# juanmc2005/diart

Measured on AMD Instinct MI355X. Metric: real-time-factor xRT streams/GPU @500ms step, higher is better.
Workload: dtype f16x3

## Files before the change

### diart_amd/_lib.py

```python
from __future__ import annotations

import ctypes as C
import os
from pathlib import Path
from typing import Optional

EXPERIMENTS = os.environ.get("DZ_EXPERIMENTS", "0") not in ("", "0")
_LIB_PATH = Path(__file__).resolve().parent / ("libdiart_amd_exp.so" if EXPERIMENTS else "libdiart_amd.so")
_lib: Optional[C.CDLL] = None

c_float_p = C.POINTER(C.c_float)
c_double_p = C.POINTER(C.c_double)
c_int_p = C.POINTER(C.c_int)
vp = C.c_void_p


class SincNetWeights(C.Structure):
    _fields_ = [("wav_gamma", C.c_float), ("wav_beta", C.c_float)] + [
        (n, vp) for n in ("filt", "in0_g", "in0_b", "w1", "b1", "in1_g", "in1_b",
                          "w2", "b2", "in2_g", "in2_b", "w1_split", "w2_split", "filt_split")]


class SegWeights(C.Structure):
    _fields_ = [("sinc", SincNetWeights), ("wih", vp * 4), ("bih", vp * 4), ("whh", vp * 4),
# ... 155 lines not shown
    "dz_tail_step": (C.c_int, [vp, vp, C.c_double, C.c_double, vp, vp, vp, vp, vp, C.c_int, vp]),
    "dz_tail_step_batch": (C.c_int, [C.POINTER(vp), C.c_int, vp, vp, vp, vp, vp, vp, vp, vp,
                                     C.c_int, vp, C.c_int]),
    "dz_file_step_batch": (C.c_int, [C.POINTER(vp), C.POINTER(vp), C.c_int, vp, vp, vp, C.c_int, C.c_int, vp, C.c_int,
                                     C.c_int, vp, C.c_double, vp, C.c_int, vp, vp, C.c_int]),
    "dz_rows_repeat": (C.c_int, [vp, vp, C.c_longlong, C.c_int, C.c_int, vp, c_int_p]),
    "dz_k_convgemm": (C.c_int, [vp, vp, vp]),
    "dz_k_gemm_f32": (C.c_int, [vp, vp, vp]),
    "dz_k_gemm_split": (C.c_int, [vp, vp, vp]),
    "dz_k_gemm_pre": (C.c_int, [vp, vp, vp]),
    "dz_k_mlp_head": (C.c_int, [vp, vp, C.c_longlong, vp, vp, vp, vp, vp, vp, C.c_int, C.c_int, C.c_int, C.c_int,
                                C.c_int, C.c_float, C.c_float, vp, vp, vp]),
    "dz_k_seg_head": (C.c_int, [vp, vp, vp, vp, C.c_int, C.c_int, C.c_int, C.c_int, C.c_int, vp, C.c_float,
                                C.c_float, C.c_int, vp, vp]),
    "dz_k_conv_pool": (C.c_int, [vp, vp, vp]),
    "dz_k_convgemm_ntile": (C.c_int, [C.c_int]),
    "dz_k_wave_stats": (C.c_int, [vp, vp, C.c_longlong, C.c_int, C.c_int, vp, vp]),
    "dz_k_sinc_conv0": (C.c_int, [vp, vp, C.c_longlong, C.c_int, C.c_int, vp, C.c_float,
                                  C.c_float, vp, vp, vp, vp]),
    "dz_k_sinc_conv0_split": (C.c_int, [vp, vp, C.c_longlong, C.c_int, C.c_int, vp, C.c_float,
                                        C.c_float, vp, vp, vp, vp]),
    "dz_k_conv0_split_ntile": (C.c_int, [C.c_int]),
    "dz_k_finalize_norm": (C.c_int, [vp, vp, C.c_int, C.c_int, C.c_int, C.c_int, vp, vp, vp, vp, vp]),
    "dz_k_lstm": (C.c_int, [vp, vp, vp, vp, C.c_int, C.c_int, vp]),
    "dz_k_lstm_mfma": (C.c_int, [vp, vp, vp, vp, C.c_int, C.c_int, C.c_int, C.c_int, vp]),
    "dz_k_lstm_planes": (C.c_int, [vp, vp, vp, vp, C.c_int, vp, C.c_longlong, C.c_int, C.c_int, vp]),
    "dz_k_stats_pool": (C.c_int, [vp, vp, C.c_int, C.c_int, C.c_int, vp, C.c_int, C.c_int,
                                  C.c_int, vp, C.c_int, vp]),
    "dz_k_powerset": (C.c_int, [vp, vp, C.c_int, C.c_int, C.c_int, vp, vp]),
    "dz_k_conv2d": (C.c_int, [vp, vp, vp, vp, vp, vp, vp, C.c_int, C.c_int, C.c_int, C.c_int, C.c_int, C.c_int,
                              C.c_int, C.c_int, vp]),
    "dz_k_ttn_depthwise": (C.c_int, [vp, vp, C.c_int, vp, C.c_int, vp, C.c_int, C.c_int, C.c_int, C.c_int, vp, vp, vp]),
}


EXPERIMENT_SIGNATURES = {
    "dz_k_gemm_g2": (C.c_int, [vp, vp, C.c_int, vp]),
    "dz_k_gemm_g3": (C.c_int, [vp, vp, C.c_int, vp]),
    "dz_k_conv_pool_debug": (C.c_int, [vp]),
    "dz_sinc_conv0_pair": (C.c_int, [vp, vp, vp, C.c_longlong, C.c_int, vp, vp, vp, vp]),
    "dz_k_sinc_conv0_pair": (C.c_int, [vp, vp, C.c_longlong, C.c_int, C.c_int, vp, vp, vp, C.c_float, C.c_float, vp, vp,
                                       vp, vp, vp]),
}


class ConvGemmDesc(C.Structure):
    _fields_ = [(n, vp) for n in ("X", "W", "bias", "e0", "e1", "nscale", "nshift", "Y", "partials")] + [
        (n, C.c_int) for n in ("B", "Tin", "Tout", "Cin", "taps", "dil", "K", "Kpad", "Npad",
                               "Nstore", "ldx", "ldy", "nld", "Tstore")] + [
        ("xbs", C.c_longlong), ("ybs", C.c_longlong), ("norm_on_load", C.c_int), ("epi", C.c_int),
        ("ksplit", C.c_int), ("ysplit", C.c_longlong), ("agroup", C.c_int), ("pad", C.c_int),
        ("X2", vp), ("rowbias", vp), ("Wsplit", vp), ("Xsplit", vp), ("xplane", C.c_longlong),
        ("Ysplit", vp), ("yplane", C.c_longlong), ("npart", vp), ("ngamma", vp), ("nbeta", vp),
        ("npart_tiles", C.c_int), ("npart_T", C.c_int), ("oflag", vp), ("Tdev", vp)]


(EPI_BIAS, EPI_BIAS_LEAKY, EPI_BIAS_SIGMOID, EPI_TDNN, EPI_POOL3, EPI_BIAS_RELU, EPI_RELU_BN,
 EPI_RELU_BN_TANH) = range(8)


class DiartAmdError(RuntimeError):
    pass


def lib_path() -> Path:
    return _LIB_PATH


def load() -> C.CDLL:
    global _lib
    if _lib is None:
        if not _LIB_PATH.exists():
            raise DiartAmdError(
                f"{_LIB_PATH} not found: build it with `python -m diart_amd.build` "
                "(hipcc, gfx950).  diart_amd has no CPU fallback.")
        lib = C.CDLL(str(_LIB_PATH))
        for name, (res, args) in SIGNATURES.items():
            fn = getattr(lib, name)
            fn.restype = res
            fn.argtypes = args
        if lib.dz_has_experiments():
            for name, (res, args) in EXPERIMENT_SIGNATURES.items():
                fn = getattr(lib, name)
                fn.restype = res
                fn.argtypes = args
        elif EXPERIMENTS:
            raise DiartAmdError(f"DZ_EXPERIMENTS=1 but {_LIB_PATH} is not an experiments build")
        sizes = (C.c_int * 5)()
        lib.dz_abi_struct_sizes(C.byref(sizes))
        mine = [C.sizeof(t) for t in (SincNetWeights, SegWeights, EmbWeights, EcapaWeights, ConvGemmDesc)]
        if list(sizes) != mine:
            raise DiartAmdError(f"{_LIB_PATH} was built from a different include/diart_amd.h: struct sizes "
                                f"{list(sizes)} (library) vs {mine} (this binding); rebuild it")
        for name, struct in (("dz_wsp", WspWeights), ("dz_sbx", SbxWeights), ("dz_ttn", TtnWeights)):
            size = getattr(lib, f"{name}_abi_size")()
            if size != C.sizeof(struct):
                raise DiartAmdError(f"{_LIB_PATH} was built from a different include/diart_amd.h: sizeof({name}_weights) "
                                    f"{size} (library) vs {C.sizeof(struct)} (this binding); rebuild it")
        _lib = lib
    return _lib


def experiments() -> bool:
    return bool(load().dz_has_experiments())


def exp_env(name: str, default: str) -> str:
# ... 47 lines not shown
```

### diart_amd/csrc/dz_embed.h

```cpp
#pragma once
#include "dz_common.h"

#include <string.h>
#include <new>

inline bool dz_conv_pool_enabled() {
    const char* v = dz_exp_env("DZ_CONV_POOL");
    return !(v && v[0] == '0');
}

struct DzGemm {
    DzConvGemm p;
    const void *wsplit, *wfrag;
    int tag, units;

    static DzGemm dense(const dz_layer& L, const float* X, int ldx, long long rows, int Cin, float* Y, int ldy,
                        int Nstore, int epi) {
        return conv1d(L, X, ldx, 1, (int)rows, Cin, Y, ldy, Nstore, epi).xstride(0, 0);
    }
    static DzGemm conv1d(const dz_layer& L, const float* X, int ldx, int B, int T, int Cin, float* Y, int ldy,
                         int Nstore, int epi) {
        DzGemm g;
        memset(&g, 0, sizeof(g));
        g.wsplit = L.wsplit;
        g.tag = -1;
        DzConvGemm& p = g.p;
        p.X = X; p.W = L.w; p.bias = L.b; p.e0 = L.s; p.e1 = L.h; p.Y = Y;
        p.B = B; p.Tin = p.Tout = p.Tstore = T; p.Cin = Cin; p.taps = 1; p.dil = 1; p.K = p.Kpad = Cin;
        p.Npad = p.Nstore = Nstore; p.ldx = ldx; p.ldy = ldy; p.epi = epi;
        return g.xstride((long long)T * ldx, (long long)T * ldy);
    }
    DzGemm& xstride(long long xbs, long long ybs) { p.xbs = xbs; p.ybs = ybs; return *this; }
    DzGemm& taps(int n, int dil, int pad) {
        p.taps = n; p.dil = dil; p.pad = pad; p.K = n * p.Cin;
        p.Tout = p.Tstore = pad ? p.Tin : p.Tin - (n - 1) * dil;
        return *this;
    }
    DzGemm& padded(int Kpad, int Npad) { p.Kpad = Kpad; p.Npad = Npad; return *this; }
    DzGemm& x2(const float* X2) { p.X2 = X2; return *this; }
    DzGemm& rowbias(const float* rb) { p.rowbias = rb; return *this; }
    DzGemm& splitk(int n, long long ysplit) { p.ksplit = n; p.ysplit = ysplit; return *this; }
    DzGemm& xplanes(const void* Xs, long long xplane) { p.Xsplit = Xs; p.xplane = Xs ? xplane : 0; return *this; }
    DzGemm& planes_out(void* Ys, long long yplane) { p.Ysplit = Ys; p.yplane = Ys ? yplane : 0; return *this; }
    DzGemm& norm_partials(const float* part, int tiles, int T, const float* gamma, const float* beta, int nld) {
        p.npart = part; p.npart_tiles = tiles; p.npart_T = T; p.ngamma = gamma; p.nbeta = beta;
        p.nld = nld; p.norm_on_load = 1;
        return *this;
    }
    DzGemm& norm_scaled(const float* nscale, const float* nshift, int nld) {
        p.nscale = nscale; p.nshift = nshift; p.nld = nld; p.norm_on_load = 1;
        return *this;
    }
    DzGemm& pool3(float* partials) {
        p.partials = partials; p.Tstore = p.Tout / 3; p.ybs = (long long)p.Tstore * p.ldy;
        return *this;
    }
    DzGemm& frag(const void* f) { wfrag = f; return *this; }
    DzGemm& tdev(const int* T) { p.Tdev = T; return *this; }
    DzGemm& prof(int t, int u) { tag = t; units = u; return *this; }

    int run(hipStream_t st) {
        DzProfScope ps(tag, units);
        if (p.Xsplit) {
            p.X = p.W = nullptr;
            p.Wsplit = wsplit;
            return dz_launch_gemm_pre(p, st);
        }
        if (wsplit && p.ksplit <= 1) {
            p.Wsplit = wsplit;
            if (p.epi == DZ_EPI_POOL3)
                return dz_conv_pool_enabled() ? dz_launch_conv_pool(p, st, wfrag) : dz_launch_gemm_split(p, st);
            p.Npad = (p.Npad + 127) / 128 * 128;
            return dz_launch_gemm_split(p, st);
        }
        DZ_REQUIRE(p.Ysplit == nullptr, "DzGemm: plane output asked of a layer that is not on the split-f16 path");
        return dz_launch_convgemm(p, st);
    }
    int run_pooled(const DzPoolFuse& q, hipStream_t st) {
        DzProfScope ps(tag, units);
        p.X = p.W = nullptr;
        p.Wsplit = wsplit;
        return dz_launch_gemm_pre_pool(p, q, st);
    }
};

constexpr int DZ_TAG_OF_GEMM = -2;
inline int dz_splitk_linear(const dz_layer& L, const float* X, int rows, int Cin, int Kpad, int N, int nsplit,
                            float* parts, int finish, float* out, hipStream_t st, int tag = -1,
// ... 90 lines not shown
```

### diart_amd/csrc/k_gemm_pre.hip

```cpp
#include "dz_common.h"
#include <stdlib.h>
#include <type_traits>

namespace {

typedef _Float16 f16x8 __attribute__((ext_vector_type(8)));
typedef _Float16 f16x2 __attribute__((ext_vector_type(2)));
typedef float f32x16 __attribute__((ext_vector_type(16)));

constexpr int BM = 128, BN = 128, KT = 32;
constexpr int PLANE_B = 128 * 64;
constexpr int plane_a(int MW) { return 64 * MW * 64; }
constexpr int stage_bytes(int MW) { return 2 * plane_a(MW) + 2 * PLANE_B; }
constexpr size_t lds_bytes(int MW) { return 2 * (size_t)stage_bytes(MW) + 3 * BN * sizeof(float); }
constexpr int MW_BIG = 6;
constexpr float LO_UNSCALE = 1.f / 2048.f;

__device__ __forceinline__ float leaky(float v) { return fmaxf(v, v * DZ_LEAKY_SLOPE); }

constexpr int YT_PITCH = 132;
constexpr int POOL_PAR = BM * YT_PITCH * 4;
constexpr int POOL_WT = POOL_PAR + 3 * BN * 4;
constexpr int POOL_RED = POOL_WT + 4 * BM * 4;
constexpr int POOL_S0 = POOL_RED + 2 * 2 * 4 * BN * 4;
constexpr size_t POOL_LDS = POOL_S0 + 8 * 8 * 2 * 4 + 8 * 2 * 4;

template <int EPI, int MW, int MT, int NT, bool ILV = false, bool POOL = false>
__device__ __forceinline__ void gemm_pre_tile(const DzConvGemm& p, const int t0, const int n0, char* smem,
                                              const int flags = 0, const DzPoolFuse* q = nullptr) {
    constexpr int PLANE_A = plane_a(MW), STAGE = stage_bytes(MW), PAR_OFF = POOL ? POOL_PAR : 2 * STAGE;
    static_assert(!POOL || (MW == 2 && MT == 2 && NT == 2), "pooled epilogue: 128 x 128 tiles only");
    const int tid = threadIdx.x;
    const int w = __builtin_amdgcn_readfirstlane(tid >> 6), l = tid & 63;

    constexpr int PA = 2 * MT * MW, PB = 4 * NT, NWAVE = 2 * MW;
    constexpr int NWA = (NWAVE * PA + (PA + PB) / 2) / (PA + PB);
    constexpr int JMAX_A = (2 * PA + NWA - 1) / NWA, JMAX_B = (2 * PB + (NWAVE - NWA) - 1) / (NWAVE - NWA);
    constexpr int JMAX = JMAX_A > JMAX_B ? JMAX_A : JMAX_B;
    const bool isB = w >= NWA;
    const int rank = isB ? w - NWA : w, group = isB ? NWAVE - NWA : NWA, npc = isB ? PB : PA;
    const unsigned short* src = isB ? reinterpret_cast<const unsigned short*>(p.Wsplit)
                                    : reinterpret_cast<const unsigned short*>(p.Xsplit);
    const int prows = isB ? p.Npad : (int)((unsigned)p.xplane / (unsigned)p.ldx);
    const long long plane_el = isB ? (long long)p.Npad * p.Kpad : p.xplane;
    const unsigned nbytes = (unsigned)((long long)prows * (isB ? p.Kpad : p.ldx) * 2);
    const __amdgpu_buffer_rsrc_t rs_hi = __builtin_amdgcn_make_buffer_rsrc((void*)src, 0, nbytes, 0x00020000);
    const __amdgpu_buffer_rsrc_t rs_lo = __builtin_amdgcn_make_buffer_rsrc((void*)(src + plane_el), 0, nbytes, 0x00020000);
    const int voff0 = ((isB ? n0 : t0) + (l >> 2)) * 64 + (((l & 3) ^ ((l >> 4) & 3)) << 4);
    constexpr int vstep = 16 * 64;
    const int kb_bytes = prows * 64;
    const int dst0 = isB ? 2 * PLANE_A : 0, dplane = isB ? PLANE_B : PLANE_A;
    auto issue = [&](int kt, int stage) {
        int cblk = kt, tap = 0;
        if (p.taps > 1) {
            cblk = kt / p.taps;
            tap = kt - cblk * p.taps;
        }
        const int soff = isB ? (tap * (p.Cin >> 5) + cblk) * kb_bytes : cblk * kb_bytes + tap * p.dil * 64;
        char* dst = smem + stage * STAGE + dst0;
#pragma unroll
        for (int j = 0; j < JMAX; ++j) {
            const int q = rank + j * group;
            if (q >= 2 * npc) break;
            const int lo = q >= npc, i = q - lo * npc;
            __builtin_amdgcn_raw_ptr_buffer_load_lds(lo ? rs_lo : rs_hi,
                (__attribute__((address_space(3))) void*)(dst + lo * dplane + i * 1024), 16,
                voff0 + i * vstep, soff, 0, 0);
        }
    };

    const int li = l & 31, g = l >> 5;
    const int wm = w >> 1, wn = w & 1;
    const int sw = (li >> 2) & 3;
    int foff[2];
#pragma unroll
    for (int ks = 0; ks < 2; ++ks) foff[ks] = li * 64 + (((2 * ks + g) ^ sw) << 4);
    f32x16 accm[MT][NT], accx[MT][NT];
#pragma unroll
    for (int mt = 0; mt < MT; ++mt)
#pragma unroll
        for (int nt = 0; nt < NT; ++nt)
#pragma unroll
            for (int r = 0; r < 16; ++r) accm[mt][nt][r] = accx[mt][nt][r] = 0.f;

    auto compute = [&](int stage) {
        const char* st = smem + stage * STAGE;
        const char* sa = st + (wm * 32 * MT) * 64;
        const char* sb = st + 2 * PLANE_A + (wn * 32 * NT) * 64;
#pragma unroll
        for (int ks = 0; ks < 2; ++ks) {
            f16x8 ah[MT], al[MT], bh[NT], bl[NT];
#pragma unroll
            for (int t = 0; t < MT; ++t) {
                ah[t] = *reinterpret_cast<const f16x8*>(sa + t * 2048 + foff[ks]);
                al[t] = *reinterpret_cast<const f16x8*>(sa + PLANE_A + t * 2048 + foff[ks]);
            }
#pragma unroll
            for (int t = 0; t < NT; ++t) {
                bh[t] = *reinterpret_cast<const f16x8*>(sb + t * 2048 + foff[ks]);
                bl[t] = *reinterpret_cast<const f16x8*>(sb + PLANE_B + t * 2048 + foff[ks]);
            }
#pragma unroll
            for (int mt = 0; mt < MT; ++mt)
#pragma unroll
                for (int nt = 0; nt < NT; ++nt) {
                    accx[mt][nt] = __builtin_amdgcn_mfma_f32_32x32x16_f16(bh[nt], al[mt], accx[mt][nt], 0, 0, 0);
                    accm[mt][nt] = __builtin_amdgcn_mfma_f32_32x32x16_f16(bh[nt], ah[mt], accm[mt][nt], 0, 0, 0);
                    accx[mt][nt] = __builtin_amdgcn_mfma_f32_32x32x16_f16(bl[nt], ah[mt], accx[mt][nt], 0, 0, 0);
                }
        }
    };

    const int nk = p.Kpad / KT;
    issue(0, 0);
    constexpr bool FULL = MW == 2 && MT == 2 && NT == 2;
    float* par = reinterpret_cast<float*>(smem + PAR_OFF);
    {
        constexpr bool AFF = EPI == DZ_EPI_TDNN || EPI == DZ_EPI_RELU_BN;
        const int which = tid >> 5, c4 = (tid & 31) * 4;
        if (which < (AFF ? 3 : 1)) {
            const float* src = which == 0 ? p.bias : which == 1 ? p.e0 : p.e1;
            f32x4 v = {0.f, 0.f, 0.f, 0.f};
            if (n0 + c4 + 3 < p.Npad) v = *reinterpret_cast<const f32x4*>(src + n0 + c4);
            *reinterpret_cast<f32x4*>(par + which * BN + c4) = v;
        }
    }
    if (FULL && ILV) {
        const int r2 = w & 1;
        char* const dbase = smem + dst0 + r2 * 1024;
        const int vofs = voff0 + r2 * vstep;
        int cblk = 0, tap = 0;
        const int tap_step = isB ? (p.Cin >> 5) * kb_bytes : p.dil * 64;
        auto advance = [&]() -> int {
            if (++tap == p.taps) { tap = 0; ++cblk; }
            return cblk * kb_bytes + tap * tap_step;
        };
        int soff_next = 0, stage_next = 0;
        const bool no_dma = flags & 2, no_rd = flags & 4;
        const bool skip_a = (flags & 32) && !isB;
        auto piece = [&](int j) {
            const int lo = j >= 4, i = r2 + 2 * (j & 3);
            (void)i;
            if (no_dma || (skip_a && tap != 0 && cblk > 0)) return;
            __builtin_amdgcn_raw_ptr_buffer_load_lds(lo ? rs_lo : rs_hi,
                (__attribute__((address_space(3))) void*)(dbase + stage_next * STAGE + lo * dplane + (j & 3) * 2048), 16,
                vofs + (j & 3) * 2 * vstep, soff_next, 0, 0);
        };
        const char* sa0 = smem + (wm * 64) * 64;
        const char* sb0 = smem + 2 * PLANE_A + (wn * 64) * 64;
#define DZ_RD(base, plane, t, ks) (*reinterpret_cast<const f16x8*>((no_rd ? smem : (base) + (plane) + (t) * 2048) + foff[ks]))
#define DZ_MM(mt, nt)                                                                                     \
    accx[mt][nt] = __builtin_amdgcn_mfma_f32_32x32x16_f16(bh[nt], al[mt], accx[mt][nt], 0, 0, 0);          \
    accm[mt][nt] = __builtin_amdgcn_mfma_f32_32x32x16_f16(bh[nt], ah[mt], accm[mt][nt], 0, 0, 0);          \
    accx[mt][nt] = __builtin_amdgcn_mfma_f32_32x32x16_f16(bl[nt], ah[mt], accx[mt][nt], 0, 0, 0)
#define DZ_PIN() __builtin_amdgcn_sched_barrier(0)
        auto body = [&](const int kt, auto more_c) {
            constexpr bool more = decltype(more_c)::value;
            asm volatile("s_waitcnt vmcnt(0) lgkmcnt(0)\n\ts_barrier" ::: "memory");
            soff_next = advance();
            stage_next = (kt + 1) & 1;
            const char* sa = sa0 + (kt & 1) * STAGE;
            const char* sb = sb0 + (kt & 1) * STAGE;
            f16x8 ah[2], al[2], bh[2], bl[2];
            bh[0] = DZ_RD(sb, 0, 0, 0); al[0] = DZ_RD(sa, PLANE_A, 0, 0); ah[0] = DZ_RD(sa, 0, 0, 0);
            bl[0] = DZ_RD(sb, PLANE_B, 0, 0);
            bh[1] = DZ_RD(sb, 0, 1, 0); bl[1] = DZ_RD(sb, PLANE_B, 1, 0);
            ah[1] = DZ_RD(sa, 0, 1, 0); al[1] = DZ_RD(sa, PLANE_A, 1, 0);
            DZ_PIN();
            accx[0][0] = __builtin_amdgcn_mfma_f32_32x32x16_f16(bh[0], al[0], accx[0][0], 0, 0, 0);
            accm[0][0] = __builtin_amdgcn_mfma_f32_32x32x16_f16(bh[0], ah[0], accm[0][0], 0, 0, 0);
            DZ_PIN();
            if (more) piece(0);
            DZ_PIN();
            accx[0][0] = __builtin_amdgcn_mfma_f32_32x32x16_f16(bl[0], ah[0], accx[0][0], 0, 0, 0);
            accx[0][1] = __builtin_amdgcn_mfma_f32_32x32x16_f16(bh[1], al[0], accx[0][1], 0, 0, 0);
            DZ_PIN();
            if (more) piece(1);
            DZ_PIN();
            accm[0][1] = __builtin_amdgcn_mfma_f32_32x32x16_f16(bh[1], ah[0], accm[0][1], 0, 0, 0);
            accx[0][1] = __builtin_amdgcn_mfma_f32_32x32x16_f16(bl[1], ah[0], accx[0][1], 0, 0, 0);
            DZ_PIN();
            if (more) piece(2);
            ah[0] = DZ_RD(sa, 0, 0, 1); al[0] = DZ_RD(sa, PLANE_A, 0, 1);
            DZ_PIN();
            accx[1][1] = __builtin_amdgcn_mfma_f32_32x32x16_f16(bh[1], al[1], accx[1][1], 0, 0, 0);
            accm[1][1] = __builtin_amdgcn_mfma_f32_32x32x16_f16(bh[1], ah[1], accm[1][1], 0, 0, 0);
            DZ_PIN();
            if (more) piece(3);
            DZ_PIN();
            accx[1][1] = __builtin_amdgcn_mfma_f32_32x32x16_f16(bl[1], ah[1], accx[1][1], 0, 0, 0);
            accx[1][0] = __builtin_amdgcn_mfma_f32_32x32x16_f16(bh[0], al[1], accx[1][0], 0, 0, 0);
            DZ_PIN();
            if (more) piece(4);
            bh[1] = DZ_RD(sb, 0, 1, 1); bl[1] = DZ_RD(sb, PLANE_B, 1, 1);
            DZ_PIN();
            accm[1][0] = __builtin_amdgcn_mfma_f32_32x32x16_f16(bh[0], ah[1], accm[1][0], 0, 0, 0);
            accx[1][0] = __builtin_amdgcn_mfma_f32_32x32x16_f16(bl[0], ah[1], accx[1][0], 0, 0, 0);
            DZ_PIN();
            if (more) piece(5);
// ... 342 lines not shown
    gemm_pre_tile<EPI, MW_BIG, 2, 2>(p, bx * 64 * MW_BIG, by * BN, smem);
}
int big_tiles_mode() {
    static const int mode = [] {
        const char* e = dz_exp_env("DZ_GEMM_BIG");
        return e ? atoi(e) : 0;
    }();
    return mode;
}

bool interleaved_loop() {
    static const bool on = [] {
        const char* e = dz_exp_env("DZ_GP_LOOP");
        return !(e && e[0] == '0');
    }();
    return on;
}

int dbg_flags() {
    static const int f = [] {
        const char* e = dz_exp_env("DZ_GP_DBG");
        return e ? atoi(e) : 0;
    }();
    return f;
}

bool tail_tiles_enabled() {
    static const bool on = [] {
        const char* e = dz_exp_env("DZ_GEMM_TAIL");
        return e && e[0] == '1';
    }();
    return on;
}
int wg_slots() {
    static const int slots = [] {
        int dev = 0, cus = 256;
        if (hipGetDevice(&dev) == hipSuccess) hipDeviceGetAttribute(&cus, hipDeviceAttributeMultiprocessorCount, dev);
        return 2 * (cus > 0 ? cus : 256);
    }();
    return slots;
}

template <int EPI>
int launch(const DzConvGemm& p, hipStream_t st) {
    static DzAttrOnce attr_ilv;
    DZ_HIP(attr_ilv.raise((const void*)gemm_pre_kernel<EPI, true>, (int)lds_bytes(2)));
    const int gx = (p.Tout + BM - 1) / BM, gy = p.Npad / BN, slots = wg_slots();
#ifdef DZ_EXPERIMENTS
    static DzAttrOnce attr_once, attr_big;
    DZ_HIP(attr_once.raise((const void*)gemm_pre_kernel<EPI, false>, (int)lds_bytes(2)));
    {
        const int gxb = (p.Tout + 64 * MW_BIG - 1) / (64 * MW_BIG);
        const int mode = big_tiles_mode();
        if (mode == 1 && gxb >= 8) {
            DZ_HIP(attr_big.raise((const void*)gemm_pre_big_kernel<EPI>, (int)lds_bytes(MW_BIG)));
            DZ_LAUNCH((gemm_pre_big_kernel<EPI>), dim3(gxb * gy), dim3(64 * 2 * MW_BIG), lds_bytes(MW_BIG), st, p);
            DZ_HIP(hipGetLastError());
            return 0;
        }
    }
#endif
    int mbig = gx;
    const int tiles = gx * gy, rem = tiles % slots;
    if (4 * tiles < slots)
        mbig = 0;
    else if (tail_tiles_enabled() && rem != 0 && 4 * rem < 3 * slots)
        mbig = (tiles / slots) * slots / gy;
    const int rows_left = p.Tout - mbig * BM;
    const int msmall = rows_left > 0 ? (rows_left + 63) / 64 : 0;
    const int nwg = mbig * gy + ((msmall + 7) / 8) * 8 * (2 * gy);
#ifdef DZ_EXPERIMENTS
    if (!interleaved_loop())
        DZ_LAUNCH((gemm_pre_kernel<EPI, false>), dim3(nwg), dim3(256), lds_bytes(2), st, p, mbig, msmall, 0);
    else
#endif
        DZ_LAUNCH((gemm_pre_kernel<EPI, true>), dim3(nwg), dim3(256), lds_bytes(2), st, p, mbig, msmall, dbg_flags());
    DZ_HIP(hipGetLastError());
    return 0;
}

}

int dz_gemm_gen() {
    static const int gen = [] {
        const char* e = dz_exp_env("DZ_GEMM_GEN");
        const int v = e ? atoi(e) : 1;
        return v == 2 || v == 3 ? v : 1;
    }();
    return gen;
}

bool dz_gemm_pre_pool_ok(const DzConvGemm& p) {
    const int gx = (p.Tout + BM - 1) / BM, gy = p.Npad / BN;
    return 4 * gx * gy >= wg_slots();
}

int dz_launch_gemm_pre_pool(const DzConvGemm& p_in, const DzPoolFuse& q, hipStream_t st) {
    DzConvGemm p = p_in;
    if (!p.oflag) p.oflag = dz_cur_oflag;
    DZ_REQUIRE(p.Wsplit && p.Xsplit && q.part && q.s0, "gemm_pre_pool: NULL operand");
    DZ_REQUIRE(p.epi == DZ_EPI_TDNN && p.B == 1 && p.taps == 1 && p.K == p.Kpad && p.Cin % KT == 0 &&
                   p.Npad % BN == 0 && p.Tout == p.Tin,
               "gemm_pre_pool: built for the flattened 1 x 1 TDNN layer");
    DZ_REQUIRE(q.np == dz_pool_pieces(q.P), "gemm_pre_pool: np must be dz_pool_pieces(P)");
    DZ_REQUIRE(q.K >= 1 && q.K <= 4 && q.P >= BM && q.T >= 2 && q.T <= q.P && p.Tout % q.P == 0 && (q.Fw >= 2 || q.Fw <= -2),
               "gemm_pre_pool: 1..4 speakers, chunk pitch >= 128 rows (got K %d, P %d, T %d)", q.K, q.P, q.T);
    DZ_REQUIRE(p.ldx > 0 && p.ldx % KT == 0 && p.xplane % p.ldx == 0 && p.xplane / p.ldx >= p.Tin,
               "gemm_pre_pool: kb-major input planes need ldx %% 32 == 0 and xplane = rows * ldx with rows >= Tin");
    DZ_REQUIRE(p.xplane * 2 < (1ll << 31) && (long long)p.Npad * p.Kpad * 2 < (1ll << 31),
               "gemm_pre_pool: operand plane exceeds the 2 GiB buffer-offset range");
    static const int pool_ag = [] {
        const char* e = dz_exp_env("DZ_POOL_AG");
        return e && atoi(e) > 0 ? atoi(e) : 1;
    }();
    if (!p.agroup) p.agroup = pool_ag;
    static DzAttrOnce attr_once;
    DZ_HIP(attr_once.raise((const void*)gemm_pre_pool_kernel, (int)POOL_LDS));
    const int gx = (p.Tout + BM - 1) / BM, gy = p.Npad / BN;
    DZ_LAUNCH(gemm_pre_pool_kernel, dim3(gx * gy), dim3(256), POOL_LDS, st, p, q, gx, dbg_flags());
    DZ_HIP(hipGetLastError());
    return 0;
}

int dz_launch_gemm_pre(const DzConvGemm& p_in, hipStream_t st) {
    DzConvGemm p = p_in;
    if (!p.oflag) p.oflag = dz_cur_oflag;
    DZ_REQUIRE(p.Wsplit != nullptr && p.Xsplit != nullptr,
               "gemm_pre: Wsplit / Xsplit (f16 hi/lo planes of W and of the input) are NULL");
    DZ_REQUIRE(p.Y != nullptr || p.Ysplit != nullptr, "gemm_pre: no output");
    DZ_REQUIRE(p.B == 1, "gemm_pre: flattened layers only (B = 1)");
    DZ_REQUIRE(p.K == p.Kpad && p.K == p.taps * p.Cin && p.Cin % KT == 0,
               "gemm_pre: K = taps * Cin without padding, Cin a multiple of 32");
    DZ_REQUIRE(p.Npad % BN == 0, "gemm_pre: Npad must be a multiple of 128");
    DZ_REQUIRE(p.Tout > 0 && p.Tout == p.Tin - (p.taps - 1) * p.dil, "gemm_pre: Tout mismatch");
    DZ_REQUIRE(p.pad == 0 && p.X2 == nullptr && p.rowbias == nullptr && p.ksplit <= 1 && !p.norm_on_load,
               "gemm_pre: padding / second input / row bias / split-K / norm-on-load are not built here");
    DZ_REQUIRE(p.ldx > 0 && p.ldx % KT == 0 && p.xplane % p.ldx == 0 && p.xplane / p.ldx >= p.Tin,
               "gemm_pre: kb-major input planes need ldx %% 32 == 0 and xplane = rows * ldx with rows >= Tin");
    DZ_REQUIRE(p.xplane * 2 < (1ll << 31) && (long long)p.Npad * p.Kpad * 2 < (1ll << 31),
               "gemm_pre: operand plane exceeds the 2 GiB buffer-offset range");
    DZ_REQUIRE(p.Ysplit == nullptr || (p.ldy > 0 && p.ldy % KT == 0 && p.yplane % p.ldy == 0 && p.yplane / p.ldy >= p.Tout &&
                                       p.Npad <= p.ldy && p.yplane * 2 < (1ll << 31)),
               "gemm_pre: kb-major output planes need ldy %% 32 == 0, yplane = rows * ldy with rows >= Tout, Npad <= ldy");
    DZ_REQUIRE(p.Y == nullptr || (p.ldy % 4 == 0 && ((uintptr_t)p.Y & 15) == 0),
               "gemm_pre: f32 output needs ldy a multiple of 4 and a 16-byte aligned base");
#ifdef DZ_EXPERIMENTS
    if (dz_gemm_gen() >= 2 && 4 * ((p.Tout + BM - 1) / BM) * (p.Npad / BN) >= wg_slots()) {
        static const int g3_min_k = [] {
            const char* e = dz_exp_env("DZ_G3_MINK");
            return e ? atoi(e) : 1024;
        }();
        if (dz_gemm_gen() == 3) {
            if (p.K >= g3_min_k) return dz_launch_gemm_g3(p, 0, st);
        } else {
            return dz_launch_gemm_g2(p, 0, st);
        }
    }
#endif
    switch (p.epi) {
        case DZ_EPI_BIAS: return launch<DZ_EPI_BIAS>(p, st);
        case DZ_EPI_BIAS_LEAKY: return launch<DZ_EPI_BIAS_LEAKY>(p, st);
        case DZ_EPI_TDNN: return launch<DZ_EPI_TDNN>(p, st);
        case DZ_EPI_RELU_BN: return launch<DZ_EPI_RELU_BN>(p, st);
    }
    dz_set_error("gemm_pre: epilogue %d is not built on the pre-split path", p.epi);
    return 2;
}
```

### diart_amd/csrc/xvec_api.hip

```cpp
#include "dz_sincnet.h"

struct dz_emb {
    dz_ctx* ctx;
    dz_emb_weights w;
    SincGeom g;
    int Bm, T[5];
    bool pre;
    const float* ext_stats;
    const float* cur_stats;
    int ext_conv0_B;
    char* arena;
    SincScratch ss;
    float *a, *b, *x5, *pooled, *parts, *ppart, *ps0;
    int pending_B;
    const float* pending_in;
};
static const int kTdnnTaps[5] = {5, 3, 3, 1, 1};
static const int kTdnnDil[5] = {1, 2, 3, 1, 1};
static const int kTdnnCin[5] = {64, 512, 512, 512, 512};
static const int kTdnnN[5] = {512, 512, 512, 512, 1536};
static const int kPoolLd = 3008;
static const int kMaxSpk = 8;
static const int kEmbSplit = 16;

extern "C" int dz_emb_frames_for(int num_samples) {
    const int f = sinc_geom(num_samples).P2 - 4 - 4 - 6;
    return f > 0 ? f : 0;
}

static void emb_carve(dz_emb* e, Arena& a) {
    e->ss.carve(a, e->g, e->Bm);
    e->a = a.take((size_t)e->Bm * e->g.P2 * 512);
    e->b = a.take((size_t)e->Bm * e->g.P2 * 512);
    e->x5 = a.take((size_t)e->Bm * e->g.P2 * 1536);
    e->pooled = a.take((size_t)e->Bm * kMaxSpk * kPoolLd);
    const int np = dz_pool_pieces(e->g.P2);
    e->ppart = a.take((size_t)e->Bm * np * 4 * 1536 * 2);
    e->ps0 = a.take((size_t)e->Bm * np * 4 * 2);
    e->parts = a.take((size_t)kEmbSplit * e->Bm * kMaxSpk * 512);
}

extern "C" int dz_emb_create(dz_ctx* ctx, const dz_emb_weights* w, int max_batch, int num_samples,
                             dz_emb** out) {
    DZ_REQUIRE(ctx && w && out, "dz_emb_create: NULL argument");
    DZ_REQUIRE(max_batch >= 1, "dz_emb_create: max_batch %d", max_batch);
    DZ_REQUIRE(w->dimension == 512, "dz_emb_create: dimension %d (only 512 is built)", w->dimension);
    const SincGeom g = sinc_geom(num_samples, w->sinc.filt_split != nullptr);
    DZ_REQUIRE(g.ok && g.P2 > 14, "dz_emb_create: %d samples is too short", num_samples);
    DZ_REQUIRE((w->sinc.w1_split != nullptr) == (w->sinc.w2_split != nullptr) &&
                   (w->sinc.w1_split != nullptr) == (w->tw_split[0] != nullptr),
               "dz_emb_create: the split planes of SincNet conv1 / conv2 and of tdnn1 must be all present "
               "or all absent (the consumer of the last SincNet stage finalises its InstanceNorm)");
    DZ_HIP(hipSetDevice(ctx->device));
    dz_emb* e = new (std::nothrow) dz_emb;
    DZ_REQUIRE(e != nullptr, "dz_emb_create: out of memory");
    e->ctx = ctx; e->w = *w; e->g = g; e->Bm = max_batch; e->arena = nullptr; e->ext_stats = nullptr; e->cur_stats = nullptr;
    e->ext_conv0_B = 0;
    e->pending_B = 0; e->pending_in = nullptr;
    e->pre = w->tw_split[0] && w->tw_split[1] && w->tw_split[2] &&
             w->tw_split[3] && w->tw_split[4];
    int t = g.P2;
    for (int i = 0; i < 5; ++i) {
        t -= (kTdnnTaps[i] - 1) * kTdnnDil[i];
        e->T[i] = t;
    }
    return sinc_handle_alloc("dz_emb_create", e, emb_carve, dz_emb_destroy, out);
}

extern "C" int dz_emb_destroy(dz_emb* emb) { return dz_handle_destroy(emb); }

extern "C" int dz_emb_use_wave_stats(dz_emb* emb, const float* d_moments) {
    DZ_REQUIRE(emb != nullptr, "dz_emb_use_wave_stats: NULL handle");
    emb->ext_stats = d_moments;
    return 0;
}

static DzGemm emb_tdnn(const dz_emb* e, int i, const void* wsplit, const float* in, bool in_planes, int B, float* out) {
    const long long rows = (long long)B * e->g.P2;
    const int cin = kTdnnCin[i], n = kTdnnN[i], K = cin * kTdnnTaps[i];
    const bool out_planes = e->pre && i < 4;
    const dz_layer L = {e->w.tw[i], e->w.tb[i], e->w.ts[i], e->w.th[i], wsplit};
    return DzGemm::dense(L, in, cin, rows, cin, out_planes ? nullptr : out, n, n, DZ_EPI_TDNN)
        .taps(kTdnnTaps[i], kTdnnDil[i], 0).padded((K + 31) / 32 * 32, n).xplanes(in_planes ? in : nullptr, rows * cin)
        .planes_out(out_planes ? out : nullptr, rows * n).prof(DZ_T_TDNN1 + i, B);
}
static DzGemm emb_tdnn5(const dz_emb* e, const float* in, int B, float* out) {
    return emb_tdnn(e, 4, e->w.tw_split[4], in, e->pre, B, out);
}

static int emb_frames(dz_emb* e, const float* d_wave, long long stride, int B, hipStream_t st) {
    const dz_emb_weights& w = e->w;
    int rc;
    const float* ext;
    bool pair;
    if ((rc = sinc_take_handoffs("dz_emb_frames", e, B, &ext, &pair))) return rc;
    const SincOut src = sinc_out_source(w.sinc, e->pre, w.tw0_split_kb);
    if ((rc = run_sincnet(w.sinc, e->g, e->ss, d_wave, stride, B, st, src, ext, pair))) return rc;
    e->cur_stats = ext ? ext : e->ss.stats;
    e->pending_B = 0;
    if (src == SINC_OUT_NORM_ON_LOAD) {
        const int P = e->g.P2;
        const dz_layer L = {w.tw[0], w.tb[0], w.ts[0], w.th[0], w.tw_split[0]};
        DzGemm g = DzGemm::conv1d(L, e->ss.y2, 64, B, P, 64, e->pre ? nullptr : e->a, 512, 512, DZ_EPI_TDNN).taps(5, 1, 0)
                       .padded(320, 512).planes_out(e->pre ? e->a : nullptr, (long long)B * P * 512).prof(DZ_T_TDNN1, B);
        rc = sinc_y2_norm(g, w.sinc, e->g, e->ss).run(st);
    } else {
        const bool planes = src == SINC_OUT_PLANES;
        rc = emb_tdnn(e, 0, planes ? w.tw0_split_kb : w.tw_split[0], e->ss.y2s, planes, B, e->a).run(st);
    }
    if (rc) return rc;
    const float* in = e->a;
    for (int i = 1; i < 4; ++i) {
        float* out = (i & 1) ? e->b : e->a;
        if ((rc = emb_tdnn(e, i, w.tw_split[i], in, e->pre, B, out).run(st))) return rc;
        in = out;
    }
    DzGemm g5 = emb_tdnn5(e, in, B, e->x5);
    if (e->pre && dz_option(DZ_OPT_POOL_FUSE) != 0 && e->g.P2 >= 128 && e->T[4] >= 2 && dz_gemm_pre_pool_ok(g5.p)) {
        e->pending_B = B;
        e->pending_in = in;
        return 0;
    }
    return g5.run(st);
}

static int emb_head(dz_emb* e, const float* d_weights, int Fw, int rows, int rows_per_x,
                    int normalize, float* d_out, hipStream_t st) {
    int rc;
    if (e->w.pool_nearest && d_weights) Fw = -Fw;
    const int nx = rows / rows_per_x, P = e->g.P2;
    bool pooled = false;
    if (e->pending_B > 0) {
        DZ_REQUIRE(nx == e->pending_B, "dz_emb_pool: %d chunks, but the frame features of %d are pending", nx,
                   e->pending_B);
        if (rows_per_x <= 4) {
            DzPoolFuse q;
            q.w = d_weights; q.Fw = Fw; q.K = rows_per_x; q.P = P; q.T = e->T[4]; q.np = dz_pool_pieces(P);
            q.part = e->ppart; q.s0 = e->ps0;
            if ((rc = emb_tdnn5(e, e->pending_in, nx, nullptr).run_pooled(q, st))) return rc;
            DzProfScope ps(DZ_T_POOL, nx);
            if ((rc = dz_launch_pool_combine(e->ppart, e->ps0, nx, rows_per_x, dz_pool_pieces(P), P, e->T[4], 1500, 1536,
                                             e->pooled, kPoolLd, st)))
                return rc;
            pooled = true;
        } else {
            if ((rc = emb_tdnn5(e, e->pending_in, nx, e->x5).run(st))) return rc;
            e->pending_B = 0;
        }
    }
    if (!pooled) {
        DzProfScope ps(DZ_T_POOL, nx);
        if ((rc = dz_launch_stats_pool(e->x5, (long long)P * 1536, e->T[4], 1500, 1536, d_weights, Fw, rows, rows_per_x,
                                       e->pooled, kPoolLd, st)))
            return rc;
    }
    const dz_layer lin = {e->w.emb_w, e->w.emb_b, nullptr, nullptr, nullptr};
    return dz_splitk_linear(lin, e->pooled, rows, kPoolLd, kPoolLd, 512, kEmbSplit, e->parts, normalize, d_out, st,
                            DZ_T_EMBLIN, DZ_T_L2, e->pre ? e->cur_stats : nullptr, rows_per_x);
}

struct EmbEntry {
    const char *who, *batch_fmt, *spk_fmt;
};
static int emb_open(const EmbEntry& en, dz_emb* e, bool have_args, int batch, int K, bool frames_ok, int weight_frames,
                    bool has_wave, const float* d_wave, long long wave_stride) {
    DZ_REQUIRE(e && have_args, "%s: NULL argument", en.who);
    DZ_REQUIRE(batch >= 1 && batch <= e->Bm, en.batch_fmt, en.who, batch, e->Bm);
    DZ_REQUIRE(K >= 1 && K <= kMaxSpk, en.spk_fmt, en.who, K, kMaxSpk);
    DZ_REQUIRE(frames_ok, "%s: weight_frames %d", en.who, weight_frames);
    if (has_wave)
        if (int rc = check_wave(en.who, d_wave, wave_stride, e->g.S)) return rc;
    DZ_HIP(hipSetDevice(e->ctx->device));
    return 0;
}

extern "C" int dz_emb_forward(dz_emb* e, const float* d_wave, long long wave_stride,
                              const float* d_weights, int n_rows, int weight_frames, float* d_out,
                              void* stream) {
    const EmbEntry en = {"dz_emb_forward", "%s: %d rows outside [1, %d]", ""};
    if (int rc = emb_open(en, e, d_out != nullptr, n_rows, 1, d_weights == nullptr || weight_frames >= 2, weight_frames,
                          true, d_wave, wave_stride))
        return rc;
    DzRangeScope range_scope(e->ctx->oflag_dev);
// ... 64 lines not shown
```

### include/diart_amd.h

```cpp
#ifndef DIART_AMD_H
#define DIART_AMD_H

#ifdef __cplusplus
extern "C" {
#endif

#define DZ_VERSION 230

typedef struct dz_ctx dz_ctx;
typedef struct dz_seg dz_seg;
typedef struct dz_emb dz_emb;
typedef struct dz_clu dz_clu;

const char* dz_last_error(void);
int dz_version(void);
int dz_set_option(const char* name, int value);
int dz_get_option(const char* name, int* value);
int dz_has_experiments(void);
int dz_host_pool_set_spin(int microseconds);

int dz_ctx_create(int hip_device, dz_ctx** out);
int dz_ctx_destroy(dz_ctx* ctx);
int dz_range_check(dz_ctx* ctx, int reset);

// ... 219 lines not shown
int dz_resample_forward(dz_resample* m, const float* d_in, long long in_stride, long long in_len, int rows,
                        float* d_out, long long out_stride, void* stream);
int dz_resample_destroy(dz_resample* m);

int dz_osp(dz_ctx* ctx, const float* d_seg, int batch, int frames, int speakers,
           float gamma, float beta, int normalize, int speaker_major,
           float* d_out, void* stream);

int dz_results_to_host(dz_ctx* ctx, const float* d_a, float* h_a, long long n_a,
                       const float* d_b, float* h_b, long long n_b, void* stream);

int dz_l2_normalize(dz_ctx* ctx, float* d_emb, int rows, int dim, float norm, void* stream);

int dz_cdist_cosine(dz_ctx* ctx, const float* d_emb, const double* d_centers,
                    int n_streams, int k_local, int g_global, int dim,
                    double* d_out, void* stream);

int dz_rows_repeat(dz_ctx* ctx, const float* d_wave, long long wave_stride, int n_rows, int num_samples,
                   void* stream, int* repeat_out);

enum { DZ_EPI_BIAS = 0, DZ_EPI_BIAS_LEAKY = 1, DZ_EPI_BIAS_SIGMOID = 2, DZ_EPI_TDNN = 3,
       DZ_EPI_POOL3 = 4, DZ_EPI_BIAS_RELU = 5, DZ_EPI_RELU_BN = 6, DZ_EPI_RELU_BN_TANH = 7 };
typedef struct {
    const float* X;
    const float* W;
    const float* bias;
    const float* e0;
    const float* e1;
    const float* nscale;
    const float* nshift;
    float* Y;
    float* partials;
    int B, Tin, Tout, Cin, taps, dil, K, Kpad, Npad, Nstore, ldx, ldy, nld, Tstore;
    long long xbs, ybs;
    int norm_on_load;
    int epi;
    int ksplit;
    long long ysplit;
    int agroup;
    int pad;
    const float* X2;
    const float* rowbias;
    const void* Wsplit;
    const void* Xsplit;
    long long xplane;
    void* Ysplit;
    long long yplane;
    const float* npart;
    const float* ngamma;
    const float* nbeta;
    int npart_tiles, npart_T;
    int* oflag;
    const int* Tdev;
} dz_convgemm_desc;
int dz_k_convgemm(dz_ctx* ctx, const dz_convgemm_desc* desc, void* stream);
int dz_k_gemm_f32(dz_ctx* ctx, const dz_convgemm_desc* desc, void* stream);
int dz_k_gemm_split(dz_ctx* ctx, const dz_convgemm_desc* desc, void* stream);
int dz_k_gemm_pre(dz_ctx* ctx, const dz_convgemm_desc* desc, void* stream);
int dz_k_mlp_head(dz_ctx* ctx, const void* xsplit, long long xplane, const void* w0split, const void* w1split,
                  const float* b0, const float* b1, const float* cw, const float* cb, int rows, int frames,
                  int classes, int speakers, int powerset, float gamma, float beta, float* d_seg,
                  float* d_weights, void* stream);
int dz_k_seg_head(dz_ctx* ctx, const float* m1, const float* cw, const float* cb, int batch, int frames,
                  int classes, int speakers, int powerset, float* d_seg, float gamma, float beta,
                  int normalize, float* d_weights, void* stream);
int dz_k_conv_pool(dz_ctx* ctx, const dz_convgemm_desc* desc, void* stream);
int dz_k_convgemm_ntile(int t_out);
int dz_k_wave_stats(dz_ctx* ctx, const float* d_wave, long long stride, int batch, int samples,
                    float* d_stats, void* stream);
int dz_k_sinc_conv0(dz_ctx* ctx, const float* d_wave, long long stride, int batch, int samples,
                    const float* d_stats, float gamma, float beta, const float* d_filt,
                    float* d_y0, float* d_partials, void* stream);
int dz_k_sinc_conv0_split(dz_ctx* ctx, const float* d_wave, long long stride, int batch, int samples,
                          const float* d_stats, float gamma, float beta, const void* d_filt_split,
                          float* d_y0, float* d_partials, void* stream);
int dz_k_conv0_split_ntile(int samples);
int dz_k_finalize_norm(dz_ctx* ctx, const float* d_partials, int batch, int ntile, int channels,
                       int frames, const float* d_gamma, const float* d_beta, float* d_scale,
                       float* d_shift, void* stream);
int dz_k_lstm(dz_ctx* ctx, const float* d_gx, const float* d_whh, float* d_hout, int batch,
              int frames, void* stream);
int dz_k_lstm_mfma(dz_ctx* ctx, const float* d_gx, const void* d_whh_split, float* d_hout,
                   int batch, int frames, int unit_major, int variant, void* stream);
int dz_k_lstm_planes(dz_ctx* ctx, const float* d_gx, const float* d_whh, const void* d_whh_split,
                     int variant, void* d_hsplit, long long hplane, int batch, int frames, void* stream);
int dz_k_stats_pool(dz_ctx* ctx, const float* d_x, int frames, int channels, int ldx,
                    const float* d_weights, int weight_frames, int rows, int rows_per_x,
                    float* d_out, int ldo, void* stream);
int dz_k_powerset(dz_ctx* ctx, const float* d_logits, int rows, int classes, int speakers,
                  float* d_out, void* stream);

int dz_clu_create(double tau_active, double rho_update, double delta_new,
                  int max_speakers, dz_clu** out);
int dz_clu_reset(dz_clu* clu);
int dz_clu_step(dz_clu* clu, const float* seg, int frames, int k_local,
                const float* emb, int dim, double* scores_out, int* assign_out);
int dz_clu_step_batch(dz_clu** clus, int n, const float* seg, int frames, int k_local,
                      const float* emb, int dim, double* scores_out, int* assign_out,
                      int num_threads);
int dz_clu_get_centers(dz_clu* clu, double* out, int dim);
int dz_clu_get_active(dz_clu* clu, int* out_mask);
int dz_clu_dim(dz_clu* clu);
int dz_clu_set_state(dz_clu* clu, const double* centers, const int* active_mask, int dim);
int dz_clu_destroy(dz_clu* clu);

int dz_prof_enable(int on);
// ... 53 lines not shown
```

Before: 33280.

## Pack TDNN layer outputs per chunk to skip invalid tail frames

The TDNN layers in the embedding stack now shrink the per-chunk row pitch from layer to layer, down to the number of valid output frames, instead of keeping the full padded pitch P2. The GEMM loader remaps each A-row index across chunk boundaries so that only valid frames are computed and stored. This cuts MMA work and memory traffic in the later layers. In exchange it adds per-row offset arithmetic in the loader, and the big-tile and gen3 kernel paths are disabled whenever packing is active.

```diff
diff --git a/diart_amd/_lib.py b/diart_amd/_lib.py
--- a/diart_amd/_lib.py
+++ b/diart_amd/_lib.py
@@ -231,7 +231,8 @@
         ("ksplit", C.c_int), ("ysplit", C.c_longlong), ("agroup", C.c_int), ("pad", C.c_int),
         ("X2", vp), ("rowbias", vp), ("Wsplit", vp), ("Xsplit", vp), ("xplane", C.c_longlong),
         ("Ysplit", vp), ("yplane", C.c_longlong), ("npart", vp), ("ngamma", vp), ("nbeta", vp),
-        ("npart_tiles", C.c_int), ("npart_T", C.c_int), ("oflag", vp), ("Tdev", vp)]
+        ("npart_tiles", C.c_int), ("npart_T", C.c_int), ("oflag", vp), ("Tdev", vp),
+        ("chunk_in", C.c_int), ("chunk_out", C.c_int)]
 
 
 (EPI_BIAS, EPI_BIAS_LEAKY, EPI_BIAS_SIGMOID, EPI_TDNN, EPI_POOL3, EPI_BIAS_RELU, EPI_RELU_BN,
diff --git a/diart_amd/csrc/dz_embed.h b/diart_amd/csrc/dz_embed.h
--- a/diart_amd/csrc/dz_embed.h
+++ b/diart_amd/csrc/dz_embed.h
@@ -34,6 +34,13 @@
     DzGemm& taps(int n, int dil, int pad) {
         p.taps = n; p.dil = dil; p.pad = pad; p.K = n * p.Cin;
         p.Tout = p.Tstore = pad ? p.Tin : p.Tin - (n - 1) * dil;
+        return *this;
+    }
+    DzGemm& chunks(int Pin, int Pout) {
+        if (Pin != Pout) {
+            p.chunk_in = Pin; p.chunk_out = Pout;
+            p.Tout = p.Tstore = p.Tin / Pin * Pout;
+        }
         return *this;
     }
     DzGemm& padded(int Kpad, int Npad) { p.Kpad = Kpad; p.Npad = Npad; return *this; }
diff --git a/diart_amd/csrc/k_gemm_pre.hip b/diart_amd/csrc/k_gemm_pre.hip
--- a/diart_amd/csrc/k_gemm_pre.hip
+++ b/diart_amd/csrc/k_gemm_pre.hip
@@ -17,6 +17,8 @@
 constexpr float LO_UNSCALE = 1.f / 2048.f;
 
 __device__ __forceinline__ float leaky(float v) { return fmaxf(v, v * DZ_LEAKY_SLOPE); }
+
+__device__ __forceinline__ int packed_row(int v, int vbnd, int vgap) { return v + (v >= vbnd ? vgap : 0); }
 
 constexpr int YT_PITCH = 132;
 constexpr int POOL_PAR = BM * YT_PITCH * 4;
@@ -46,7 +48,14 @@
     const unsigned nbytes = (unsigned)((long long)prows * (isB ? p.Kpad : p.ldx) * 2);
     const __amdgpu_buffer_rsrc_t rs_hi = __builtin_amdgcn_make_buffer_rsrc((void*)src, 0, nbytes, 0x00020000);
     const __amdgpu_buffer_rsrc_t rs_lo = __builtin_amdgcn_make_buffer_rsrc((void*)(src + plane_el), 0, nbytes, 0x00020000);
-    const int voff0 = ((isB ? n0 : t0) + (l >> 2)) * 64 + (((l & 3) ^ ((l >> 4) & 3)) << 4);
+    int voff0 = ((isB ? n0 : t0) + (l >> 2)) * 64 + (((l & 3) ^ ((l >> 4) & 3)) << 4);
+    int vbnd = 0x7fffffff, vgap = 0;
+    if (!POOL && p.chunk_in != p.chunk_out && !isB) {
+        const int b0 = __builtin_amdgcn_readfirstlane(t0 / p.chunk_out), d = p.chunk_in - p.chunk_out;
+        voff0 += b0 * d * 64;
+        vbnd = ((b0 + 1) * p.chunk_out + b0 * d) * 64;
+        vgap = d * 64;
+    }
     constexpr int vstep = 16 * 64;
     const int kb_bytes = prows * 64;
     const int dst0 = isB ? 2 * PLANE_A : 0, dplane = isB ? PLANE_B : PLANE_A;
@@ -65,7 +74,7 @@
             const int lo = q >= npc, i = q - lo * npc;
             __builtin_amdgcn_raw_ptr_buffer_load_lds(lo ? rs_lo : rs_hi,
                 (__attribute__((address_space(3))) void*)(dst + lo * dplane + i * 1024), 16,
-                voff0 + i * vstep, soff, 0, 0);
+                packed_row(voff0 + i * vstep, vbnd, vgap), soff, 0, 0);
         }
     };
 
@@ -144,7 +153,7 @@
             if (no_dma || (skip_a && tap != 0 && cblk > 0)) return;
             __builtin_amdgcn_raw_ptr_buffer_load_lds(lo ? rs_lo : rs_hi,
                 (__attribute__((address_space(3))) void*)(dbase + stage_next * STAGE + lo * dplane + (j & 3) * 2048), 16,
-                vofs + (j & 3) * 2 * vstep, soff_next, 0, 0);
+                packed_row(vofs + (j & 3) * 2 * vstep, vbnd, vgap), soff_next, 0, 0);
         };
         const char* sa0 = smem + (wm * 64) * 64;
         const char* sb0 = smem + 2 * PLANE_A + (wn * 64) * 64;
@@ -593,7 +602,7 @@
     {
         const int gxb = (p.Tout + 64 * MW_BIG - 1) / (64 * MW_BIG);
         const int mode = big_tiles_mode();
-        if (mode == 1 && gxb >= 8) {
+        if (mode == 1 && gxb >= 8 && p.chunk_in == p.chunk_out) {
             DZ_HIP(attr_big.raise((const void*)gemm_pre_big_kernel<EPI>, (int)lds_bytes(MW_BIG)));
             DZ_LAUNCH((gemm_pre_big_kernel<EPI>), dim3(gxb * gy), dim3(64 * 2 * MW_BIG), lds_bytes(MW_BIG), st, p);
             DZ_HIP(hipGetLastError());
@@ -641,7 +650,7 @@
     if (!p.oflag) p.oflag = dz_cur_oflag;
     DZ_REQUIRE(p.Wsplit && p.Xsplit && q.part && q.s0, "gemm_pre_pool: NULL operand");
     DZ_REQUIRE(p.epi == DZ_EPI_TDNN && p.B == 1 && p.taps == 1 && p.K == p.Kpad && p.Cin % KT == 0 &&
-                   p.Npad % BN == 0 && p.Tout == p.Tin,
+                   p.Npad % BN == 0 && p.Tout == p.Tin && p.chunk_in == p.chunk_out,
                "gemm_pre_pool: built for the flattened 1 x 1 TDNN layer");
     DZ_REQUIRE(q.np == dz_pool_pieces(q.P), "gemm_pre_pool: np must be dz_pool_pieces(P)");
     DZ_REQUIRE(q.K >= 1 && q.K <= 4 && q.P >= BM && q.T >= 2 && q.T <= q.P && p.Tout % q.P == 0 && (q.Fw >= 2 || q.Fw <= -2),
@@ -673,7 +682,17 @@
     DZ_REQUIRE(p.K == p.Kpad && p.K == p.taps * p.Cin && p.Cin % KT == 0,
                "gemm_pre: K = taps * Cin without padding, Cin a multiple of 32");
     DZ_REQUIRE(p.Npad % BN == 0, "gemm_pre: Npad must be a multiple of 128");
-    DZ_REQUIRE(p.Tout > 0 && p.Tout == p.Tin - (p.taps - 1) * p.dil, "gemm_pre: Tout mismatch");
+    const bool packed = p.chunk_in != p.chunk_out;
+    if (packed) {
+        DZ_REQUIRE(p.chunk_out >= BM && p.chunk_out + (p.taps - 1) * p.dil <= p.chunk_in && p.Tin % p.chunk_in == 0 &&
+                       p.Tout == p.Tin / p.chunk_in * p.chunk_out,
+                   "gemm_pre: packed chunks need 128 <= chunk_out <= chunk_in - (taps - 1) * dil, Tin = n * chunk_in and "
+                   "Tout = n * chunk_out (got chunk_in %d, chunk_out %d, Tin %d, Tout %d)", p.chunk_in, p.chunk_out, p.Tin,
+                   p.Tout);
+    } else {
+        DZ_REQUIRE(p.Tout > 0 && p.Tout == p.Tin - (p.taps - 1) * p.dil, "gemm_pre: Tout mismatch");
+        p.chunk_in = p.chunk_out = 0;
+    }
     DZ_REQUIRE(p.pad == 0 && p.X2 == nullptr && p.rowbias == nullptr && p.ksplit <= 1 && !p.norm_on_load,
                "gemm_pre: padding / second input / row bias / split-K / norm-on-load are not built here");
     DZ_REQUIRE(p.ldx > 0 && p.ldx % KT == 0 && p.xplane % p.ldx == 0 && p.xplane / p.ldx >= p.Tin,
@@ -686,7 +705,7 @@
     DZ_REQUIRE(p.Y == nullptr || (p.ldy % 4 == 0 && ((uintptr_t)p.Y & 15) == 0),
                "gemm_pre: f32 output needs ldy a multiple of 4 and a 16-byte aligned base");
 #ifdef DZ_EXPERIMENTS
-    if (dz_gemm_gen() >= 2 && 4 * ((p.Tout + BM - 1) / BM) * (p.Npad / BN) >= wg_slots()) {
+    if (!packed && dz_gemm_gen() >= 2 && 4 * ((p.Tout + BM - 1) / BM) * (p.Npad / BN) >= wg_slots()) {
         static const int g3_min_k = [] {
             const char* e = dz_exp_env("DZ_G3_MINK");
             return e ? atoi(e) : 1024;
diff --git a/diart_amd/csrc/xvec_api.hip b/diart_amd/csrc/xvec_api.hip
--- a/diart_amd/csrc/xvec_api.hip
+++ b/diart_amd/csrc/xvec_api.hip
@@ -14,6 +14,7 @@
     float *a, *b, *x5, *pooled, *parts, *ppart, *ps0;
     int pending_B;
     const float* pending_in;
+    int pitch;
 };
 static const int kTdnnTaps[5] = {5, 3, 3, 1, 1};
 static const int kTdnnDil[5] = {1, 2, 3, 1, 1};
@@ -56,7 +57,7 @@
     DZ_REQUIRE(e != nullptr, "dz_emb_create: out of memory");
     e->ctx = ctx; e->w = *w; e->g = g; e->Bm = max_batch; e->arena = nullptr; e->ext_stats = nullptr; e->cur_stats = nullptr;
     e->ext_conv0_B = 0;
-    e->pending_B = 0; e->pending_in = nullptr;
+    e->pending_B = 0; e->pending_in = nullptr; e->pitch = g.P2;
     e->pre = w->tw_split[0] && w->tw_split[1] && w->tw_split[2] &&
              w->tw_split[3] && w->tw_split[4];
     int t = g.P2;
@@ -75,17 +76,23 @@
     return 0;
 }
 
-static DzGemm emb_tdnn(const dz_emb* e, int i, const void* wsplit, const float* in, bool in_planes, int B, float* out) {
-    const long long rows = (long long)B * e->g.P2;
+static int emb_pitch(const dz_emb* e, int i, bool in_planes, int pin) {
+    return e->pre && in_planes && e->T[i] >= 128 ? e->T[i] : pin;
+}
+static DzGemm emb_tdnn(const dz_emb* e, int i, const void* wsplit, const float* in, bool in_planes, int B, int pin,
+                       float* out) {
+    const int pout = emb_pitch(e, i, in_planes, pin);
+    const long long rows = (long long)B * pin, rows_out = (long long)B * pout;
     const int cin = kTdnnCin[i], n = kTdnnN[i], K = cin * kTdnnTaps[i];
     const bool out_planes = e->pre && i < 4;
     const dz_layer L = {e->w.tw[i], e->w.tb[i], e->w.ts[i], e->w.th[i], wsplit};
     return DzGemm::dense(L, in, cin, rows, cin, out_planes ? nullptr : out, n, n, DZ_EPI_TDNN)
-        .taps(kTdnnTaps[i], kTdnnDil[i], 0).padded((K + 31) / 32 * 32, n).xplanes(in_planes ? in : nullptr, rows * cin)
-        .planes_out(out_planes ? out : nullptr, rows * n).prof(DZ_T_TDNN1 + i, B);
+        .taps(kTdnnTaps[i], kTdnnDil[i], 0).chunks(pin, pout).padded((K + 31) / 32 * 32, n)
+        .xplanes(in_planes ? in : nullptr, rows * cin).planes_out(out_planes ? out : nullptr, rows_out * n)
+        .prof(DZ_T_TDNN1 + i, B);
 }
 static DzGemm emb_tdnn5(const dz_emb* e, const float* in, int B, float* out) {
-    return emb_tdnn(e, 4, e->w.tw_split[4], in, e->pre, B, out);
+    return emb_tdnn(e, 4, e->w.tw_split[4], in, e->pre, B, e->pitch, out);
 }
 
 static int emb_frames(dz_emb* e, const float* d_wave, long long stride, int B, hipStream_t st) {
@@ -98,6 +105,7 @@
     if ((rc = run_sincnet(w.sinc, e->g, e->ss, d_wave, stride, B, st, src, ext, pair))) return rc;
     e->cur_stats = ext ? ext : e->ss.stats;
     e->pending_B = 0;
+    int pitch = e->g.P2;
     if (src == SINC_OUT_NORM_ON_LOAD) {
         const int P = e->g.P2;
         const dz_layer L = {w.tw[0], w.tb[0], w.ts[0], w.th[0], w.tw_split[0]};
@@ -106,17 +114,20 @@
         rc = sinc_y2_norm(g, w.sinc, e->g, e->ss).run(st);
     } else {
         const bool planes = src == SINC_OUT_PLANES;
-        rc = emb_tdnn(e, 0, planes ? w.tw0_split_kb : w.tw_split[0], e->ss.y2s, planes, B, e->a).run(st);
+        rc = emb_tdnn(e, 0, planes ? w.tw0_split_kb : w.tw_split[0], e->ss.y2s, planes, B, pitch, e->a).run(st);
+        pitch = emb_pitch(e, 0, planes, pitch);
     }
     if (rc) return rc;
     const float* in = e->a;
     for (int i = 1; i < 4; ++i) {
         float* out = (i & 1) ? e->b : e->a;
-        if ((rc = emb_tdnn(e, i, w.tw_split[i], in, e->pre, B, out).run(st))) return rc;
+        if ((rc = emb_tdnn(e, i, w.tw_split[i], in, e->pre, B, pitch, out).run(st))) return rc;
+        pitch = emb_pitch(e, i, e->pre, pitch);
         in = out;
     }
+    e->pitch = pitch;
     DzGemm g5 = emb_tdnn5(e, in, B, e->x5);
-    if (e->pre && dz_option(DZ_OPT_POOL_FUSE) != 0 && e->g.P2 >= 128 && e->T[4] >= 2 && dz_gemm_pre_pool_ok(g5.p)) {
+    if (e->pre && dz_option(DZ_OPT_POOL_FUSE) != 0 && e->pitch >= 128 && e->T[4] >= 2 && dz_gemm_pre_pool_ok(g5.p)) {
         e->pending_B = B;
         e->pending_in = in;
         return 0;
@@ -128,7 +139,7 @@
                     int normalize, float* d_out, hipStream_t st) {
     int rc;
     if (e->w.pool_nearest && d_weights) Fw = -Fw;
-    const int nx = rows / rows_per_x, P = e->g.P2;
+    const int nx = rows / rows_per_x, P = e->pitch;
     bool pooled = false;
     if (e->pending_B > 0) {
         DZ_REQUIRE(nx == e->pending_B, "dz_emb_pool: %d chunks, but the frame features of %d are pending", nx,
diff --git a/include/diart_amd.h b/include/diart_amd.h
--- a/include/diart_amd.h
+++ b/include/diart_amd.h
@@ -295,6 +295,7 @@
     int npart_tiles, npart_T;
     int* oflag;
     const int* Tdev;
+    int chunk_in, chunk_out;
 } dz_convgemm_desc;
 int dz_k_convgemm(dz_ctx* ctx, const dz_convgemm_desc* desc, void* stream);
 int dz_k_gemm_f32(dz_ctx* ctx, const dz_convgemm_desc* desc, void* stream);
```

After: 33220, median of 2. No clear change (-0.2%).
